# luo-yining/CFDBench

Hardware: NVIDIA H100
Metric: fno_rollout_steps_per_sec (higher is better)
Workload: dtype bf16

## Files before the change

cfdbench_b200/_lib.py:

```python
from __future__ import annotations

import ctypes as C
import os

_HERE = os.path.dirname(os.path.abspath(__file__))
LIB_PATH = os.path.join(_HERE, "libcfdbench_b200.so")

FNO_MAX_LAYERS = 8
ABI_VERSION = 4
ACT_F32, ACT_BF16 = 0, 1
EPI_GELU, EPI_GELU_SAVE_PRE, EPI_MUL_DGELU, EPI_PLAIN = 0, 1, 2, 3


class FnoWeights(C.Structure):
    _fields_ = [
        ("n_layers", C.c_int32),
        ("n_case_params", C.c_int32),
        ("fc0_w", C.c_void_p),
        ("fc0_b", C.c_void_p),
        ("spec_wk", C.c_void_p * FNO_MAX_LAYERS),
        ("w0t", C.c_void_p * FNO_MAX_LAYERS),
        ("w0_b", C.c_void_p * FNO_MAX_LAYERS),
        ("fc1_w", C.c_void_p),
        ("fc1_b", C.c_void_p),
# ... 64 lines not shown
    "fno_bwd_partials_bytes": (C.c_size_t, []),
    "fno_mode_mix_image": (C.c_int, [_P, _P, _P, _I, _P]),
    "fno_block_fused": (C.c_int, [_P, _P, _P, _P, _P, _I, _P]),
    "fno_pack_spectral_weights": (C.c_int, [_P, _P, _P, _I, _P]),
    "fno_unpack_spectral_grads": (C.c_int, [_P, _P, _P, _P]),
    "fno_mix_operand_bytes": (C.c_size_t, []),
    "fno_pack_mix_operand": (C.c_int, [_P, _P, _P]),
    "fno_pack_mix_operand_from_weights": (C.c_int, [_P, _P, _P, _I, _P]),
    "fno_lift_fwd": (C.c_int, [_P, _P, _P, C.POINTER(FnoWeights), _P, _I, _I, _P]),
    "fno_spectral_dft_fwd": (C.c_int, [_P, _P, _I, _I, _F, _F, _P]),
    "fno_mode_mix": (C.c_int, [_P, _P, _P, _I, _P]),
    "fno_spectral_inv_kx": (C.c_int, [_P, _P, _I, _F, _F, _P]),
    "fno_block_out": (C.c_int, [_I, _P, _P, _P, _P, _P, _P, _P, _I, _I, _P]),
    "fno_block_fwd": (C.c_int, [C.POINTER(FnoWeights), _I, _P, _P, _P, C.POINTER(FnoWorkspace), _I, _I, _P]),
    "fno_project_fwd": (C.c_int, [_P, _P, C.POINTER(FnoWeights), _P, _I, _I, _P]),
    "fno_forward": (C.c_int, [C.POINTER(FnoWeights), _P, _P, _P, _P, C.POINTER(FnoWorkspace), _I, _I, _P]),
    "fno_rollout": (C.c_int, [C.POINTER(FnoWeights), _P, _P, _P, _P, _I, C.POINTER(FnoWorkspace), _I, _I, _P]),
    "fno_rollout_host": (C.c_int, [C.POINTER(FnoWeights), _P, _P, _P, _P, _I, C.POINTER(FnoWorkspace), _P, _I, _I, _P]),
    "fno_rollout_host_scratch_bytes": (C.c_size_t, [_I, _I, _I]),
    "fno_multistep_metrics": (C.c_int, [_P, _P, _P, _P, _I, _I, _P]),
    "fno_gather_batch": (C.c_int, [_P, _P, _P, _P, _P, _I, _I, _I, _P, _P, _P, _P, _P]),
    "fno_loss_scratch_bytes": (C.c_size_t, []),
    "fno_loss_fwd": (C.c_int, [_P, _P, C.c_size_t, _P, _P, _P]),
    "fno_loss_bwd": (C.c_int, [_P, _P, _P, _P, _P, C.c_size_t, _P]),
    "fno_adam_step": (C.c_int, [C.POINTER(FnoAdamTensors), C.c_float, C.c_float, C.c_float, C.c_float, C.c_float,
                                C.c_int64, _P]),
    "fno_forward_train": (C.c_int, [C.POINTER(FnoWeights), _P, _P, _P, _P, C.POINTER(FnoTrainSaved),
                                    C.POINTER(FnoWorkspace), _I, _I, _P]),
    "fno_backward": (C.c_int, [C.POINTER(FnoWeights), C.POINTER(FnoWeightsBwd), _P, _P, _P, _P,
                               C.POINTER(FnoTrainSaved), C.POINTER(FnoGrads), C.POINTER(FnoBwdScratch),
# ... 55 lines not shown
```

cfdbench_b200/build.py:

```python
from __future__ import annotations

import hashlib
import os
import subprocess
import sys
import time

HERE = os.path.dirname(os.path.abspath(__file__))
CSRC = os.path.join(HERE, "csrc")
OUT = os.path.join(HERE, "libcfdbench_b200.so")
STAMP = os.path.join(HERE, ".build_stamp")
SOURCES = ["fno_abi.cu", "fno_dft_fwd.cu", "fno_dft_fwd_tc.cu", "fno_mode_mix.cu", "fno_block_tc.cu", "fno_block_fused.cu", "fno_pointwise.cu", "fno_project_tc.cu", "fno_project_bwd_tc.cu",
           "fno_backward.cu", "fno_metrics.cu", "fno_train_step.cu", "fno_grid.cu"]
NVCC_FLAGS = ["-std=c++17", "-O3", "-lineinfo", "-gencode", "arch=compute_90a,code=sm_90a",
              "-Xcompiler", "-fPIC"]


def _nvcc() -> str:
    for cand in (os.environ.get("NVCC"), "/usr/local/cuda/bin/nvcc"):
        if cand and os.path.exists(cand):
            return cand
    return "nvcc"


def _fingerprint() -> str:
    h = hashlib.sha256()
    for root in (CSRC, os.path.join(os.path.dirname(HERE), "include")):
# ... 52 lines not shown
```

cfdbench_b200/csrc/fno_abi.cu:

```cuda
#include <stdio.h>
#include <string.h>

#include "../../include/cfdbench_b200.h"
#include "fno_common.cuh"

namespace fno {
cudaError_t launch_dft_fwd(const void*, void*, int, float, float, cudaStream_t);
cudaError_t launch_mode_mix(const void*, const void*, void*, void*, int, cudaStream_t);
cudaError_t launch_block_fused(const void*, const void*, const float*, const float*, void*, int, cudaStream_t);
size_t ym_image_bytes(int);
cudaError_t launch_pack_spectral(const void*, const void*, void*, int, cudaStream_t);
cudaError_t launch_unpack_spectral(const void*, void*, void*, cudaStream_t);
cudaError_t launch_dft_fwd_tc(const void*, void*, int, float, float, cudaStream_t);
cudaError_t launch_pack_mix_operand(const void*, void*, cudaStream_t);
cudaError_t launch_pack_mix_operand_direct(const void*, const void*, void*, int, cudaStream_t);
size_t mix_operand_bytes();
cudaError_t launch_gather_batch(const void*, const void*, const float*, const int*, const long long*, int, int, int, float*,
                                float*, float*, float*, cudaStream_t);
cudaError_t launch_loss_fwd(const float*, const float*, size_t, float*, float*, cudaStream_t);
cudaError_t launch_loss_bwd(const float*, const float*, const float*, const float*, float*, size_t, cudaStream_t);
size_t loss_scratch_bytes();
cudaError_t launch_adam_step(const fno_adam_tensors*, float, float, float, float, float, long long, cudaStream_t);
cudaError_t launch_inv_kx(const void*, void*, int, float, float, cudaStream_t);
template <typename TAct>
cudaError_t launch_block_tc(int, const void*, const void*, const float*, const float*, void*, float*, const float*, int,
                            cudaStream_t);
template <typename TAct>
cudaError_t launch_lift(const float*, const float*, const float*, const float*, const float*, const float*,
                        const float*, void*, int, int, cudaStream_t);
template <typename TAct>
cudaError_t launch_project_tc(const void*, const float*, const float*, const float*, const float*, const float*,
                              float*, int, cudaStream_t);
int project_bwd_rows_max();
int project_bwd_row();
cudaError_t launch_reduce_partials(const float*, int, int, float*, int, float*, int, float*, int, int, cudaStream_t);
template <typename TAct>
cudaError_t launch_project_bwd_tc(const void*, const float*, const float*, const float*, const float*, const float*, const float*,
                                  float*, float*, float*, int*, int, cudaStream_t);
template <typename TP, typename TQ, int NJ, int NI>
cudaError_t launch_chan_outer(const void*, const void*, float*, int*, int, cudaStream_t);
cudaError_t launch_multistep_metrics(const float*, const float*, const float*, float*, int, int, cudaStream_t);
cudaError_t launch_spectral_wgrad(const void*, const void*, void*, int, cudaStream_t);
cudaError_t launch_lift_bwd(const float*, const float*, const float*, const float*, const float*, const float*,
                            float*, float*, float*, int, int, cudaStream_t);
cudaError_t launch_lift_bwd_data(const float*, const float*, float*, float*, int, int, cudaStream_t);
bool grid_ok(int, int);
void grid_tables_release(int);
// ... 178 lines not shown
  }
  FNO_TRY(fno_mode_mix(ws->xm, w->spec_wk[layer], ws->ym, batch, stream));
  const float inv = 1.f / static_cast<float>(kHW);
  FNO_TRY(fno_spectral_inv_kx(ws->ym, ws->z, batch, inv, 2.f * inv, stream));
  return fno_block_out(pre_out ? FNO_EPI_GELU_SAVE_PRE : FNO_EPI_GELU, ws->z, act_in, w->w0t[layer], w->w0_b[layer],
                       act_out, pre_out, nullptr, batch, act_dtype, stream);
}

int fno_project_fwd(const void* act_in, const float* mask, const fno_weights* w, float* preds, int batch,
                    int act_dtype, void* stream) {
  if (!act_in || !mask || !w || !preds || batch <= 0 || bad_dtype(act_dtype))
    return fail(kErrArg, "fno_project_fwd: bad argument");
  cudaError_t e =
      act_dtype == FNO_ACT_F32
          ? launch_project_tc<float>(act_in, w->fc1_w, w->fc1_b, w->fc2_w, w->fc2_b, mask, preds, batch, S(stream))
          : launch_project_tc<__nv_bfloat16>(act_in, w->fc1_w, w->fc1_b, w->fc2_w, w->fc2_b, mask, preds, batch, S(stream));
  FNO_CUDA(e, "project_kernel");
  return kOk;
}

int fno_forward(const fno_weights* w, const float* inputs, const float* mask, const float* case_params,
                float* preds, const fno_workspace* ws, int batch, int act_dtype, void* stream) {
  if (!w || !ws || !ws->act[0] || !ws->act[1] || !ws->xm) return fail(kErrArg, "fno_forward: bad workspace");
  if (!(act_dtype == FNO_ACT_BF16 && ws->ym_img) && (!ws->ym || !ws->z)) return fail(kErrArg, "fno_forward: bad workspace");
  if (w->n_layers < 1 || w->n_layers > FNO_MAX_LAYERS) return fail(kErrUnsupported, "fno_forward: n_layers out of range");
  FNO_TRY(fno_lift_fwd(inputs, mask, case_params, w, ws->act[0], batch, act_dtype, stream));
  int cur = 0;
  for (int l = 0; l < w->n_layers; ++l) {
    FNO_TRY(fno_block_fwd(w, l, ws->act[cur], ws->act[cur ^ 1], nullptr, ws, batch, act_dtype, stream));
    cur ^= 1;
  }
  return fno_project_fwd(ws->act[cur], mask, w, preds, batch, act_dtype, stream);
}

int fno_rollout(const fno_weights* w, const float* inputs, const float* mask, const float* case_params,
                float* preds_seq, int steps, const fno_workspace* ws, int batch, int act_dtype, void* stream) {
  if (steps < 0 || !preds_seq) return fail(kErrArg, "fno_rollout: bad argument");
  const size_t frame = static_cast<size_t>(batch) * 2 * kHW;
  const float* cur = inputs;
  for (int s = 0; s < steps; ++s) {
    float* nxt = preds_seq + static_cast<size_t>(s) * frame;
    FNO_TRY(fno_forward(w, cur, mask, case_params, nxt, ws, batch, act_dtype, stream));
    cur = nxt;
  }
  return kOk;
}

size_t fno_rollout_host_scratch_bytes(int batch, int n_case_params, int steps) {
  const size_t b = static_cast<size_t>(batch);
  return (b * 2 * kHW + b * kHW + static_cast<size_t>(steps) * b * 2 * kHW) * sizeof(float) +
         ((b * n_case_params * sizeof(float) + 255) / 256) * 256;
}

int fno_rollout_host(const fno_weights* w, const float* inputs_host, const float* mask_host,
                     const float* case_params_host, float* preds_seq_host, int steps, const fno_workspace* ws,
                     void* dev_io, int batch, int act_dtype, void* stream) {
  if (!w || !inputs_host || !mask_host || !preds_seq_host || !dev_io || batch <= 0 || steps <= 0)
    return fail(kErrArg, "fno_rollout_host: bad argument");
// ... 399 lines not shown
```

cfdbench_b200/csrc/fno_block_fused.cu:

```cuda
#include "fno_common.cuh"
#include "tc_common.cuh"
#include "tc_tma.cuh"
#include <math.h>
#include <string.h>

namespace fno {

constexpr int kFzRows = 16;
constexpr int kFzChunks = kH / kFzRows;
constexpr int kFzWgRows = kFzRows / 2;
constexpr int kFzThreads = 9 * 32;
constexpr int kFzProdWarp = 8;
constexpr int kZK = 2 * kM2;
constexpr int kImgK = 2 * kKX;
constexpr size_t kYmImgBytes = 147456;
constexpr uint32_t kFzStage = 4 * 6144;
constexpr int kFzFFloats = 2 * (2 * kFzRows) * kImgK;
constexpr int kFzEFloats = 2 * kW * kZK;
constexpr uint32_t kFzZtFloats = kC * kZK;
constexpr uint32_t kLboF = (2 * kFzRows / 8) * 128;
constexpr uint32_t kLboE = (kW / 8) * 128;
constexpr uint32_t kLboO = (kC / 8) * 128;
constexpr uint32_t kFzBoxW = kW, kFzBoxH = 1, kFzBoxC = kC;
constexpr uint32_t kFzRowBytes = kFzBoxW * kFzBoxH * kFzBoxC * 2;
// ... 7 lines not shown
  alignas(1024) unsigned char x[2][kFzXSlots][kFzRowBytes];
  alignas(1024) unsigned char st[2][2][kFzRowBytes];
  alignas(128) unsigned char y[2][kFzStage];
  alignas(128) float zt[kFzRows][2][kFzZtFloats];
  alignas(128) float f_hi[kFzFFloats / 2];
  alignas(128) float f_lo[kFzFFloats / 2];
  alignas(128) float e_hi[kFzEFloats / 2];
  alignas(128) float e_lo[kFzEFloats / 2];
  alignas(128) unsigned char w0[3][kFzW0Bytes];
  alignas(16) float bias[kC];
  alignas(8) uint64_t y_full[2], y_free[2];
  alignas(8) uint64_t x_full[2][kFzXSlots];
};
static_assert(sizeof(FzSmem) <= 232448, "block_fused_kernel: shared memory over the per-block opt-in limit");

__device__ __forceinline__ uint32_t sw128_bf16_offset(int line, int e) {
  return static_cast<uint32_t>(line * 128 + ((((e >> 3) ^ line) & 7) << 4) + (e & 7) * 2);
}

__global__ void __launch_bounds__(kFzThreads, 1)
    block_fused_kernel(const __grid_constant__ CUtensorMap x_map, const __grid_constant__ CUtensorMap out_map,
                       const unsigned char* __restrict__ img, const float* __restrict__ w0t,
                       const float* __restrict__ bias, const float* __restrict__ etab, const float* __restrict__ ftab,
                       int batch) {
  extern __shared__ __align__(1024) unsigned char smem_raw[];
  FzSmem& sm = *reinterpret_cast<FzSmem*>(smem_raw);
  if ((smem_u32(smem_raw) & 1023u) != 0) __trap();
  const int tid = threadIdx.x, lane = tid & 31, warp = tc::warp_index_uniform();
  const int chunk = blockIdx.x % kFzChunks, b0 = blockIdx.x / kFzChunks, bstride = gridDim.x / kFzChunks;
  const int n_units = b0 < batch ? (batch - b0 + bstride - 1) / bstride : 0;

  if (tid == 0) {
    for (int i = 0; i < 2; ++i) {
      mbar_init(&sm.y_full[i], 1);
// ... 260 lines not shown
```

cfdbench_b200/csrc/fno_project_tc.cu:

```cuda
#include "fno_common.cuh"
#include "tc_common.cuh"

namespace fno {

constexpr int kPtWG = 4;
constexpr int kPtThreads = 128 * kPtWG;
constexpr int kPtM = kW;
constexpr uint32_t kPtLboA = (kPtM / 8) * 128;
constexpr uint32_t kPtLboB = (kProj / 8) * 128;
constexpr int kPtTilesPerSample = kH;
constexpr int kPtReps = kPtM * (kC / 4) / 128;

struct PtSmem {
  alignas(128) float w_hi[kProj * kC];
  alignas(128) float w_lo[kProj * kC];
  alignas(128) float a_hi[kPtWG][kPtM * kC];
  alignas(128) float a_lo[kPtWG][kPtM * kC];
  alignas(16) float4 w2q[kProj / 2];
  alignas(16) float2 b1p[kProj / 2];
};

template <typename TAct>
struct PtRegs {
  TAct v[kPtReps][4];
};

template <typename TAct>
__device__ __forceinline__ void pt_prefetch(PtRegs<TAct>& r, const TAct* __restrict__ a, int tile, int t) {
  const int b = tile / kPtTilesPerSample, p0 = (tile % kPtTilesPerSample) * kPtM;
#pragma unroll
  for (int rep = 0; rep < kPtReps; ++rep) {
    const int task = rep * 128 + t;
    const int m = task & (kPtM - 1), kq = task >> 6;
    const TAct* src = a + (static_cast<size_t>(b) * kC + 4 * kq) * kHW + p0 + m;
#pragma unroll
    for (int c = 0; c < 4; ++c) r.v[rep][c] = __ldg(src + static_cast<size_t>(c) * kHW);
  }
}

__device__ __forceinline__ float pt_to_float(float v) { return v; }
__device__ __forceinline__ float pt_to_float(__nv_bfloat16 v) { return __bfloat162float(v); }

template <typename TAct>
__device__ __forceinline__ void pt_split_store(const PtRegs<TAct>& r, float* a_hi, float* a_lo, int t) {
#pragma unroll
  for (int rep = 0; rep < kPtReps; ++rep) {
    const int task = rep * 128 + t;
    const int m = task & (kPtM - 1), kq = task >> 6;
    float hi[4], lo[4];
#pragma unroll
    for (int c = 0; c < 4; ++c) {
      const float x = pt_to_float(r.v[rep][c]);
      if constexpr (sizeof(TAct) == 4) tc::split_tf32(x, hi[c], lo[c]);
      else hi[c] = x;
    }
    const uint32_t off = tc::kmajor_offset(m, 4 * kq, kPtM) / 4;
    *reinterpret_cast<float4*>(a_hi + off) = make_float4(hi[0], hi[1], hi[2], hi[3]);
    if constexpr (sizeof(TAct) == 4) *reinterpret_cast<float4*>(a_lo + off) = make_float4(lo[0], lo[1], lo[2], lo[3]);
  }
}

template <typename TAct>
__global__ void __launch_bounds__(kPtThreads, 1)
    project_tc_kernel(const TAct* __restrict__ a, const float* __restrict__ w1, const float* __restrict__ b1,
                      const float* __restrict__ w2, const float* __restrict__ b2, const float* __restrict__ mask,
                      float* __restrict__ preds, int n_tiles) {
  constexpr bool kBf16 = sizeof(TAct) == 2;
  extern __shared__ __align__(1024) unsigned char smem_raw[];
  PtSmem& sm = *reinterpret_cast<PtSmem*>(smem_raw);
  const int tid = threadIdx.x, lane = tid & 31;
  const int wg = tc::warp_index_uniform() >> 2, t = tid & 127, wq = (tid >> 5) & 3;

  for (int e = tid; e < kProj * kC; e += kPtThreads) {
    const int j = e / kC, i = e % kC;
    float hi, lo;
    tc::split_tf32(w1[e], hi, lo);
    const uint32_t off = tc::kmajor_offset(j, i, kProj) / 4;
    sm.w_hi[off] = hi;
    sm.w_lo[off] = lo;
  }
  if (tid < kProj / 2) {
    sm.w2q[tid] = make_float4(w2[2 * tid], w2[kProj + 2 * tid], w2[2 * tid + 1], w2[kProj + 2 * tid + 1]);
// ... 10 lines not shown
  float* a_lo = sm.a_lo[wg];
  PtRegs<TAct> regs;
  if (first < n_tiles) pt_prefetch<TAct>(regs, a, first, t);
  for (int tile = first; tile < n_tiles; tile += stride) {
    pt_split_store<TAct>(regs, a_hi, a_lo, t);
    tc::fence_proxy_async_smem();
    tc::named_barrier(1 + wg, 128);
    if (tile + stride < n_tiles) pt_prefetch<TAct>(regs, a, tile + stride, t);
    float acc[64];
    tc::wg_fence();
    {
      const uint32_t a_s[3] = {tc::smem_addr(a_hi), tc::smem_addr(a_lo), tc::smem_addr(a_hi)};
      const uint32_t b_s[3] = {tc::smem_addr(sm.w_hi), tc::smem_addr(sm.w_hi), tc::smem_addr(sm.w_lo)};
#pragma unroll
      for (int pass = 0; pass < 3; ++pass) {
        if (kBf16 && pass == 1) continue;
#pragma unroll
        for (int ks = 0; ks < kC / 8; ++ks)
          tc::wg_tf32_ss_n128(acc, tc::make_smem_desc(a_s[pass] + ks * 2 * kPtLboA, kPtLboA, 128),
                              tc::make_smem_desc(b_s[pass] + ks * 2 * kPtLboB, kPtLboB, 128), (pass | ks) ? 1u : 0u);
      }
    }
    tc::wg_commit();
    tc::wg_wait<0>();
    tc::wg_fence_acc(acc);
    const int b = tile / kPtTilesPerSample, p0 = (tile % kPtTilesPerSample) * kPtM;
#pragma unroll
    for (int hh = 0; hh < 2; ++hh) {
      float2 out = make_float2(0.f, 0.f);
#pragma unroll
      for (int i0 = 0; i0 < 16; i0 += 8) {
        float2 g[8];
#pragma unroll
        for (int i = 0; i < 8; ++i) {
          const float2 bb = sm.b1p[4 * (i0 + i) + (lane & 3)];
          g[i] = make_float2(acc[4 * (i0 + i) + 2 * hh] + bb.x, acc[4 * (i0 + i) + 2 * hh + 1] + bb.y);
        }
        if constexpr (kBf16) {
          gelu_erf2_deg5_batch<8>(g);
        } else {
#pragma unroll
          for (int i = 0; i < 8; ++i) g[i] = gelu_erf2(g[i]);
        }
#pragma unroll
        for (int i = 0; i < 8; ++i) {
          const float4 wq4 = sm.w2q[4 * (i0 + i) + (lane & 3)];
          out = ffma2(make_float2(g[i].x, g[i].x), make_float2(wq4.x, wq4.y), out);
          out = ffma2(make_float2(g[i].y, g[i].y), make_float2(wq4.z, wq4.w), out);
        }
      }
      out.x += __shfl_xor_sync(0xffffffffu, out.x, 1);
      out.y += __shfl_xor_sync(0xffffffffu, out.y, 1);
      out.x += __shfl_xor_sync(0xffffffffu, out.x, 2);
      out.y += __shfl_xor_sync(0xffffffffu, out.y, 2);
      if ((lane & 3) == 0) {
        const int pix = p0 + 16 * wq + (lane >> 2) + 8 * hh;
        const float mk = __ldg(mask + static_cast<size_t>(b) * kHW + pix);
        preds[(static_cast<size_t>(b) * 2 + 0) * kHW + pix] = (b2x + out.x) * mk;
// ... 8 lines not shown
                              const float* mask, float* preds, int batch, cudaStream_t stream) {
  auto kern = project_tc_kernel<TAct>;
  constexpr size_t smem = sizeof(PtSmem);
  static PerDeviceLaunch pd;
  int n_sm = 0;
  cudaError_t e0 = per_device_setup(kern, smem, pd, &n_sm);
  if (e0 != cudaSuccess) return e0;
  const int n_tiles = batch * kPtTilesPerSample;
  const int want = (n_tiles + kPtWG - 1) / kPtWG;
  const int grid = want < n_sm ? want : n_sm;
  return launch_chained(kern, dim3(grid), dim3(kPtThreads), smem, stream, static_cast<const TAct*>(a), w1, b1, w2, b2,
                        mask, preds, n_tiles);
}
template cudaError_t launch_project_tc<float>(const void*, const float*, const float*, const float*, const float*,
                                              const float*, float*, int, cudaStream_t);
template cudaError_t launch_project_tc<__nv_bfloat16>(const void*, const float*, const float*, const float*,
                                                      const float*, const float*, float*, int, cudaStream_t);

}
```

cfdbench_b200/csrc/tc_common.cuh:

```cuda
#pragma once
#include <cuda_runtime.h>
#include <stdint.h>

namespace fno {
namespace tc {

__device__ __forceinline__ uint32_t smem_addr(const void* p) {
  return static_cast<uint32_t>(__cvta_generic_to_shared(p));
}

__device__ __forceinline__ int warp_index_uniform() {
  return __shfl_sync(0xffffffffu, static_cast<int>(threadIdx.x >> 5), 0);
}

__device__ __forceinline__ void named_barrier(int id, int count) {
  asm volatile("bar.sync %0, %1;" ::"r"(id), "r"(count) : "memory");
}

__device__ __forceinline__ void fence_proxy_async_smem() {
  asm volatile("fence.proxy.async.shared::cta;" ::: "memory");
}

__device__ __forceinline__ uint64_t make_smem_desc(uint32_t saddr, uint32_t lbo_bytes, uint32_t sbo_bytes) {
  uint64_t d = 0;
// ... 47 lines not shown
  asm volatile(
      "{\n.reg .pred p;\nsetp.ne.b32 p, %38, 0;\n"
      "wgmma.mma_async.sync.aligned.m64n72k16.f32.bf16.bf16 {%0, %1, %2, %3, %4, %5, %6, %7, %8, %9, %10, %11, %12, %13, %14, %15, %16, %17, %18, %19, %20, %21, %22, %23, %24, %25, %26, %27, %28, %29, %30, %31, %32, %33, %34, %35}, %36, %37, p, 1, 1, 0, 0;\n}\n"
      : "+f"(d[0]), "+f"(d[1]), "+f"(d[2]), "+f"(d[3]), "+f"(d[4]), "+f"(d[5]), "+f"(d[6]), "+f"(d[7]), "+f"(d[8]), "+f"(d[9]), "+f"(d[10]), "+f"(d[11]), "+f"(d[12]), "+f"(d[13]), "+f"(d[14]), "+f"(d[15]), "+f"(d[16]), "+f"(d[17]), "+f"(d[18]), "+f"(d[19]), "+f"(d[20]), "+f"(d[21]), "+f"(d[22]), "+f"(d[23]), "+f"(d[24]), "+f"(d[25]), "+f"(d[26]), "+f"(d[27]), "+f"(d[28]), "+f"(d[29]), "+f"(d[30]), "+f"(d[31]), "+f"(d[32]), "+f"(d[33]), "+f"(d[34]), "+f"(d[35])
      : "l"(a), "l"(b), "r"(acc)
      : "memory");
}
__device__ __forceinline__ void wg_bf16_ss_n32_mn_a(float* d, uint64_t a, uint64_t b, uint32_t acc) {
  asm volatile(
      "{\n.reg .pred p;\nsetp.ne.b32 p, %18, 0;\n"
      "wgmma.mma_async.sync.aligned.m64n32k16.f32.bf16.bf16 {%0, %1, %2, %3, %4, %5, %6, %7, %8, %9, %10, %11, %12, %13, %14, %15}, %16, %17, p, 1, 1, 1, 0;\n}\n"
      : "+f"(d[0]), "+f"(d[1]), "+f"(d[2]), "+f"(d[3]), "+f"(d[4]), "+f"(d[5]), "+f"(d[6]), "+f"(d[7]), "+f"(d[8]), "+f"(d[9]), "+f"(d[10]), "+f"(d[11]), "+f"(d[12]), "+f"(d[13]), "+f"(d[14]), "+f"(d[15])
      : "l"(a), "l"(b), "r"(acc)
      : "memory");
}
__device__ __forceinline__ void wg_tf32_rs_n32(float* d, const uint32_t* a, uint64_t b, uint32_t acc) {
  asm volatile(
      "{\n.reg .pred p;\nsetp.ne.b32 p, %21, 0;\n"
      "wgmma.mma_async.sync.aligned.m64n32k8.f32.tf32.tf32 {%0, %1, %2, %3, %4, %5, %6, %7, %8, %9, %10, %11, %12, %13, %14, %15}, {%16, %17, %18, %19}, %20, p, 1, 1;\n}\n"
      : "+f"(d[0]), "+f"(d[1]), "+f"(d[2]), "+f"(d[3]), "+f"(d[4]), "+f"(d[5]), "+f"(d[6]), "+f"(d[7]), "+f"(d[8]), "+f"(d[9]), "+f"(d[10]), "+f"(d[11]), "+f"(d[12]), "+f"(d[13]), "+f"(d[14]), "+f"(d[15])
      : "r"(a[0]), "r"(a[1]), "r"(a[2]), "r"(a[3]), "l"(b), "r"(acc)
      : "memory");
}
__device__ __forceinline__ void wg_tf32_rs_n64(float* d, const uint32_t* a, uint64_t b, uint32_t acc) {
  asm volatile(
      "{\n.reg .pred p;\nsetp.ne.b32 p, %37, 0;\n"
      "wgmma.mma_async.sync.aligned.m64n64k8.f32.tf32.tf32 {%0, %1, %2, %3, %4, %5, %6, %7, %8, %9, %10, %11, %12, %13, %14, %15, %16, %17, %18, %19, %20, %21, %22, %23, %24, %25, %26, %27, %28, %29, %30, %31}, {%32, %33, %34, %35}, %36, p, 1, 1;\n}\n"
      : "+f"(d[0]), "+f"(d[1]), "+f"(d[2]), "+f"(d[3]), "+f"(d[4]), "+f"(d[5]), "+f"(d[6]), "+f"(d[7]), "+f"(d[8]), "+f"(d[9]), "+f"(d[10]), "+f"(d[11]), "+f"(d[12]), "+f"(d[13]), "+f"(d[14]), "+f"(d[15]), "+f"(d[16]), "+f"(d[17]), "+f"(d[18]), "+f"(d[19]), "+f"(d[20]), "+f"(d[21]), "+f"(d[22]), "+f"(d[23]), "+f"(d[24]), "+f"(d[25]), "+f"(d[26]), "+f"(d[27]), "+f"(d[28]), "+f"(d[29]), "+f"(d[30]), "+f"(d[31])
      : "r"(a[0]), "r"(a[1]), "r"(a[2]), "r"(a[3]), "l"(b), "r"(acc)
      : "memory");
// ... 16 lines not shown
```

cfdbench_b200/csrc/tc_tma.cuh:

```cuda
#pragma once
#include "fno_common.cuh"
#include <cuda.h>

namespace fno {

__device__ __forceinline__ void tma_load_2d(void* dst, const CUtensorMap* tm, int c0, int c1, uint64_t* bar) {
  asm volatile("cp.async.bulk.tensor.2d.shared::cluster.global.mbarrier::complete_tx::bytes [%0], [%1, {%2, %3}], [%4];" ::"r"(
                   smem_u32(dst)),
               "l"(tm), "r"(c0), "r"(c1), "r"(smem_u32(bar))
               : "memory");
}
__device__ __forceinline__ void tma_load_3d(void* dst, const CUtensorMap* tm, int c0, int c1, int c2, uint64_t* bar) {
  asm volatile(
      "cp.async.bulk.tensor.3d.shared::cluster.global.mbarrier::complete_tx::bytes [%0], [%1, {%2, %3, %4}], [%5];" ::"r"(
          smem_u32(dst)),
      "l"(tm), "r"(c0), "r"(c1), "r"(c2), "r"(smem_u32(bar))
      : "memory");
}
__device__ __forceinline__ void tma_store_3d(const CUtensorMap* tm, const void* src, int c0, int c1, int c2) {
  asm volatile("cp.async.bulk.tensor.3d.global.shared::cta.bulk_group [%0, {%2, %3, %4}], [%1];" ::"l"(tm),
               "r"(smem_u32(src)), "r"(c0), "r"(c1), "r"(c2)
               : "memory");
}
__device__ __forceinline__ void bulk_commit_group() { asm volatile("cp.async.bulk.commit_group;" ::: "memory"); }
template <int kPending>
__device__ __forceinline__ void bulk_wait_group_read() {
  asm volatile("cp.async.bulk.wait_group.read %0;" ::"n"(kPending) : "memory");
}
template <int kPending>
__device__ __forceinline__ void bulk_wait_group() {
  asm volatile("cp.async.bulk.wait_group %0;" ::"n"(kPending) : "memory");
}

typedef CUresult (*TmaEncodeFn)(CUtensorMap*, CUtensorMapDataType, cuuint32_t, void*, const cuuint64_t*, const cuuint64_t*,
                                const cuuint32_t*, const cuuint32_t*, CUtensorMapInterleave, CUtensorMapSwizzle,
                                CUtensorMapL2promotion, CUtensorMapFloatOOBfill);
inline cudaError_t tma_encode_fn(TmaEncodeFn* out) {
// ... 41 lines not shown
```

include/cfdbench_b200.h:

```cpp
#ifndef CFDBENCH_B200_H_
#define CFDBENCH_B200_H_

#include <stddef.h>
#include <stdint.h>

#ifdef __cplusplus
extern "C" {
#endif

#define FNO_ABI_VERSION 4
#define FNO_MAX_LAYERS 8

enum { FNO_ACT_F32 = 0, FNO_ACT_BF16 = 1 };
enum { FNO_EPI_GELU = 0, FNO_EPI_GELU_SAVE_PRE = 1, FNO_EPI_MUL_DGELU = 2, FNO_EPI_PLAIN = 3 };

typedef struct fno_weights {
  int32_t n_layers;
  int32_t n_case_params;
  const float* fc0_w;
  const float* fc0_b;
  const void* spec_wk[FNO_MAX_LAYERS];
  const float* w0t[FNO_MAX_LAYERS];
  const float* w0_b[FNO_MAX_LAYERS];
  const float* fc1_w;
// ... 32 lines not shown
                 void* act_out, int batch, int act_dtype, void* stream);

int fno_spectral_dft_fwd(const void* act_in, void* xm, int batch, int act_dtype, float s0, float s1, void* stream);
int fno_mode_mix(const void* xm, const void* wop, void* ym, int batch, void* stream);
int fno_spectral_inv_kx(const void* ym, void* z, int batch, float s0, float s1, void* stream);
int fno_block_out(int epilogue, const void* z, const void* act_in, const float* w0t, const float* bias, void* act_out,
                  float* pre_out, const float* pre_in, int batch, int act_dtype, void* stream);
int fno_mode_mix_image(const void* xm, const void* wop, void* ym_img, int batch, void* stream);
int fno_block_fused(const void* ym_img, const void* act_in_bf16, const float* w0t, const float* bias, void* act_out_bf16,
                    int batch, void* stream);
int fno_block_fwd(const fno_weights* w, int layer, const void* act_in, void* act_out, float* pre_out,
                  const fno_workspace* ws, int batch, int act_dtype, void* stream);

int fno_project_fwd(const void* act_in, const float* mask, const fno_weights* w, float* preds, int batch,
                    int act_dtype, void* stream);

int fno_forward(const fno_weights* w, const float* inputs, const float* mask, const float* case_params,
                float* preds, const fno_workspace* ws, int batch, int act_dtype, void* stream);

int fno_rollout(const fno_weights* w, const float* inputs, const float* mask, const float* case_params,
                float* preds_seq, int steps, const fno_workspace* ws, int batch, int act_dtype, void* stream);

int fno_rollout_host(const fno_weights* w, const float* inputs_host, const float* mask_host,
                     const float* case_params_host, float* preds_seq_host, int steps, const fno_workspace* ws,
                     void* dev_io, int batch, int act_dtype, void* stream);
size_t fno_rollout_host_scratch_bytes(int batch, int n_case_params, int steps);


typedef struct fno_train_saved {
  void* act[FNO_MAX_LAYERS + 1];
// ... 103 lines not shown
```

Before: 1211.

## Fuse bf16 projection with next-step lift in rollout via new wgmma kernel

Adds a bf16 projection kernel that uses TMA-loaded activation rows and bf16 wgmma with a 3-term split of fc1 weights. In rollout, the kernel also computes the next step's lifted activation directly from its predictions, removing a separate lift launch and the round trip through global memory for each step. The bf16 path of the old TF32 projection kernel is removed and replaced by the new kernel. This adds kernel complexity, and the triple-bf16 weight split risks small numeric differences.

```diff
diff --git a/cfdbench_b200/_lib.py b/cfdbench_b200/_lib.py
--- a/cfdbench_b200/_lib.py
+++ b/cfdbench_b200/_lib.py
@@ -102,6 +102,7 @@
     "fno_block_out": (C.c_int, [_I, _P, _P, _P, _P, _P, _P, _P, _I, _I, _P]),
     "fno_block_fwd": (C.c_int, [C.POINTER(FnoWeights), _I, _P, _P, _P, C.POINTER(FnoWorkspace), _I, _I, _P]),
     "fno_project_fwd": (C.c_int, [_P, _P, C.POINTER(FnoWeights), _P, _I, _I, _P]),
+    "fno_project_lift_fwd": (C.c_int, [_P, _P, _P, C.POINTER(FnoWeights), _P, _P, _I, _P]),
     "fno_forward": (C.c_int, [C.POINTER(FnoWeights), _P, _P, _P, _P, C.POINTER(FnoWorkspace), _I, _I, _P]),
     "fno_rollout": (C.c_int, [C.POINTER(FnoWeights), _P, _P, _P, _P, _I, C.POINTER(FnoWorkspace), _I, _I, _P]),
     "fno_rollout_host": (C.c_int, [C.POINTER(FnoWeights), _P, _P, _P, _P, _I, C.POINTER(FnoWorkspace), _P, _I, _I, _P]),
diff --git a/cfdbench_b200/build.py b/cfdbench_b200/build.py
--- a/cfdbench_b200/build.py
+++ b/cfdbench_b200/build.py
@@ -10,7 +10,7 @@
 CSRC = os.path.join(HERE, "csrc")
 OUT = os.path.join(HERE, "libcfdbench_b200.so")
 STAMP = os.path.join(HERE, ".build_stamp")
-SOURCES = ["fno_abi.cu", "fno_dft_fwd.cu", "fno_dft_fwd_tc.cu", "fno_mode_mix.cu", "fno_block_tc.cu", "fno_block_fused.cu", "fno_pointwise.cu", "fno_project_tc.cu", "fno_project_bwd_tc.cu",
+SOURCES = ["fno_abi.cu", "fno_dft_fwd.cu", "fno_dft_fwd_tc.cu", "fno_mode_mix.cu", "fno_block_tc.cu", "fno_block_fused.cu", "fno_pointwise.cu", "fno_project_tc.cu", "fno_project_bf16.cu", "fno_project_bwd_tc.cu",
            "fno_backward.cu", "fno_metrics.cu", "fno_train_step.cu", "fno_grid.cu"]
 NVCC_FLAGS = ["-std=c++17", "-O3", "-lineinfo", "-gencode", "arch=compute_90a,code=sm_90a",
               "-Xcompiler", "-fPIC"]
diff --git a/cfdbench_b200/csrc/fno_abi.cu b/cfdbench_b200/csrc/fno_abi.cu
--- a/cfdbench_b200/csrc/fno_abi.cu
+++ b/cfdbench_b200/csrc/fno_abi.cu
@@ -31,6 +31,9 @@
 template <typename TAct>
 cudaError_t launch_project_tc(const void*, const float*, const float*, const float*, const float*, const float*,
                               float*, int, cudaStream_t);
+cudaError_t launch_project_bf16(const void*, const float*, const float*, const float*, const float*, const float*, float*,
+                                void*, const float*, const float*, const float*, const float*, const float*, int, int,
+                                cudaStream_t);
 int project_bwd_rows_max();
 int project_bwd_row();
 cudaError_t launch_reduce_partials(const float*, int, int, float*, int, float*, int, float*, int, int, cudaStream_t);
@@ -239,22 +242,57 @@
   cudaError_t e =
       act_dtype == FNO_ACT_F32
           ? launch_project_tc<float>(act_in, w->fc1_w, w->fc1_b, w->fc2_w, w->fc2_b, mask, preds, batch, S(stream))
-          : launch_project_tc<__nv_bfloat16>(act_in, w->fc1_w, w->fc1_b, w->fc2_w, w->fc2_b, mask, preds, batch, S(stream));
-  FNO_CUDA(e, "project_kernel");
-  return kOk;
-}
-
-int fno_forward(const fno_weights* w, const float* inputs, const float* mask, const float* case_params,
-                float* preds, const fno_workspace* ws, int batch, int act_dtype, void* stream) {
-  if (!w || !ws || !ws->act[0] || !ws->act[1] || !ws->xm) return fail(kErrArg, "fno_forward: bad workspace");
-  if (!(act_dtype == FNO_ACT_BF16 && ws->ym_img) && (!ws->ym || !ws->z)) return fail(kErrArg, "fno_forward: bad workspace");
-  if (w->n_layers < 1 || w->n_layers > FNO_MAX_LAYERS) return fail(kErrUnsupported, "fno_forward: n_layers out of range");
-  FNO_TRY(fno_lift_fwd(inputs, mask, case_params, w, ws->act[0], batch, act_dtype, stream));
-  int cur = 0;
+          : launch_project_bf16(act_in, w->fc1_w, w->fc1_b, w->fc2_w, w->fc2_b, mask, preds, nullptr, nullptr, nullptr,
+                                nullptr, nullptr, nullptr, 0, batch, S(stream));
+  FNO_CUDA(e, act_dtype == FNO_ACT_F32 ? "project_tc_kernel" : "project_bf16_kernel");
+  return kOk;
+}
+
+int fno_project_lift_fwd(const void* act_in, const float* mask, const float* case_params, const fno_weights* w, float* preds,
+                         void* act_next, int batch, void* stream) {
+  if (!act_in || !mask || !w || !preds || !act_next || batch <= 0 || !w->gx || !w->gy)
+    return fail(kErrArg, "fno_project_lift_fwd: bad argument");
+  if (w->n_case_params < 0 || w->n_case_params > kMaxCaseParams)
+    return fail(kErrArg, "fno_project_lift_fwd: n_case_params out of range");
+  if (w->n_case_params > 0 && !case_params) return fail(kErrArg, "fno_project_lift_fwd: case_params is null");
+  if ((reinterpret_cast<uintptr_t>(act_in) | reinterpret_cast<uintptr_t>(act_next)) & 15)
+    return fail(kErrArg, "fno_project_lift_fwd: act_in / act_next must be 16-byte aligned");
+  const size_t bytes = fno_act_bytes(batch, FNO_ACT_BF16);
+  const char *in = static_cast<const char*>(act_in), *nx = static_cast<const char*>(act_next);
+  if (in < nx + bytes && nx < in + bytes) return fail(kErrArg, "fno_project_lift_fwd: act_in and act_next overlap");
+  FNO_CUDA(launch_project_bf16(act_in, w->fc1_w, w->fc1_b, w->fc2_w, w->fc2_b, mask, preds, act_next, case_params, w->fc0_w,
+                               w->fc0_b, w->gx, w->gy, w->n_case_params, batch, S(stream)),
+           "project_bf16_kernel(lift)");
+  return kOk;
+}
+
+static int check_forward_workspace(const char* what, const fno_weights* w, const fno_workspace* ws, int act_dtype) {
+  char msg[128];
+  snprintf(msg, sizeof(msg), "%s: bad workspace", what);
+  if (!w || !ws || !ws->act[0] || !ws->act[1] || !ws->xm) return fail(kErrArg, msg);
+  if (!(act_dtype == FNO_ACT_BF16 && ws->ym_img) && (!ws->ym || !ws->z)) return fail(kErrArg, msg);
+  snprintf(msg, sizeof(msg), "%s: n_layers out of range", what);
+  if (w->n_layers < 1 || w->n_layers > FNO_MAX_LAYERS) return fail(kErrUnsupported, msg);
+  return kOk;
+}
+
+static int forward_layers(const fno_weights* w, const fno_workspace* ws, int a0, int batch, int act_dtype, void* stream,
+                          int* out) {
+  int cur = a0;
   for (int l = 0; l < w->n_layers; ++l) {
     FNO_TRY(fno_block_fwd(w, l, ws->act[cur], ws->act[cur ^ 1], nullptr, ws, batch, act_dtype, stream));
     cur ^= 1;
   }
+  *out = cur;
+  return kOk;
+}
+
+int fno_forward(const fno_weights* w, const float* inputs, const float* mask, const float* case_params,
+                float* preds, const fno_workspace* ws, int batch, int act_dtype, void* stream) {
+  FNO_TRY(check_forward_workspace("fno_forward", w, ws, act_dtype));
+  FNO_TRY(fno_lift_fwd(inputs, mask, case_params, w, ws->act[0], batch, act_dtype, stream));
+  int cur = 0;
+  FNO_TRY(forward_layers(w, ws, 0, batch, act_dtype, stream, &cur));
   return fno_project_fwd(ws->act[cur], mask, w, preds, batch, act_dtype, stream);
 }
 
@@ -262,11 +300,26 @@
                 float* preds_seq, int steps, const fno_workspace* ws, int batch, int act_dtype, void* stream) {
   if (steps < 0 || !preds_seq) return fail(kErrArg, "fno_rollout: bad argument");
   const size_t frame = static_cast<size_t>(batch) * 2 * kHW;
-  const float* cur = inputs;
+  if (act_dtype != FNO_ACT_BF16) {
+    const float* cur = inputs;
+    for (int s = 0; s < steps; ++s) {
+      float* nxt = preds_seq + static_cast<size_t>(s) * frame;
+      FNO_TRY(fno_forward(w, cur, mask, case_params, nxt, ws, batch, act_dtype, stream));
+      cur = nxt;
+    }
+    return kOk;
+  }
+  if (steps == 0) return kOk;
+  FNO_TRY(check_forward_workspace("fno_rollout", w, ws, act_dtype));
+  FNO_TRY(fno_lift_fwd(inputs, mask, case_params, w, ws->act[0], batch, act_dtype, stream));
+  int a0 = 0;
   for (int s = 0; s < steps; ++s) {
     float* nxt = preds_seq + static_cast<size_t>(s) * frame;
-    FNO_TRY(fno_forward(w, cur, mask, case_params, nxt, ws, batch, act_dtype, stream));
-    cur = nxt;
+    int cur = 0;
+    FNO_TRY(forward_layers(w, ws, a0, batch, act_dtype, stream, &cur));
+    if (s + 1 == steps) return fno_project_fwd(ws->act[cur], mask, w, nxt, batch, act_dtype, stream);
+    FNO_TRY(fno_project_lift_fwd(ws->act[cur], mask, case_params, w, nxt, ws->act[cur ^ 1], batch, stream));
+    a0 = cur ^ 1;
   }
   return kOk;
 }
diff --git a/cfdbench_b200/csrc/fno_block_fused.cu b/cfdbench_b200/csrc/fno_block_fused.cu
--- a/cfdbench_b200/csrc/fno_block_fused.cu
+++ b/cfdbench_b200/csrc/fno_block_fused.cu
@@ -45,10 +45,6 @@
 };
 static_assert(sizeof(FzSmem) <= 232448, "block_fused_kernel: shared memory over the per-block opt-in limit");
 
-__device__ __forceinline__ uint32_t sw128_bf16_offset(int line, int e) {
-  return static_cast<uint32_t>(line * 128 + ((((e >> 3) ^ line) & 7) << 4) + (e & 7) * 2);
-}
-
 __global__ void __launch_bounds__(kFzThreads, 1)
     block_fused_kernel(const __grid_constant__ CUtensorMap x_map, const __grid_constant__ CUtensorMap out_map,
                        const unsigned char* __restrict__ img, const float* __restrict__ w0t,
diff --git a/cfdbench_b200/csrc/fno_project_bf16.cu b/cfdbench_b200/csrc/fno_project_bf16.cu
--- /dev/null
+++ b/cfdbench_b200/csrc/fno_project_bf16.cu
@@ -0,0 +1,264 @@
+#include "fno_common.cuh"
+#include "tc_common.cuh"
+#include "tc_tma.cuh"
+#include <type_traits>
+
+namespace fno {
+
+constexpr int kPjWG = 4;
+constexpr int kPjThreads = 128 * kPjWG;
+constexpr int kPjTilesPerSample = kH;
+constexpr uint32_t kPjBoxW = kW, kPjBoxH = 1, kPjBoxC = kC;
+constexpr uint32_t kPjRowBytes = kPjBoxW * kPjBoxH * kPjBoxC * 2;
+constexpr int kPjXSlots = 4;
+constexpr uint32_t kPjW1Bytes = kProj * kC * 2;
+constexpr uint32_t kPjLboW = (kProj / 8) * 128;
+
+__host__ __device__ constexpr int pj_x_slot(int n) { return n % kPjXSlots; }
+__host__ __device__ constexpr uint32_t pj_x_parity(int n) { return static_cast<uint32_t>(n / kPjXSlots) & 1u; }
+
+struct PjSmem {
+  alignas(1024) unsigned char x[kPjWG][kPjXSlots][kPjRowBytes];
+  alignas(1024) unsigned char st[kPjWG][2][kPjRowBytes];
+  alignas(128) unsigned char w1[3][kPjW1Bytes];
+  alignas(16) float4 w2q[kProj / 2];
+  alignas(16) float2 b1p[kProj / 2];
+  alignas(16) float4 lw4[kC];
+  float lwx[kC];
+  float lwp[kC][kMaxCaseParams];
+  float lb[kC];
+  float gx[kH], gy[kW];
+  float base[kPjWG][2][kC];
+  alignas(8) uint64_t x_full[kPjWG][kPjXSlots];
+};
+static_assert(sizeof(PjSmem) <= 232448, "project_bf16_kernel: shared memory over the per-block opt-in limit");
+
+template <bool kLift>
+__global__ void __launch_bounds__(kPjThreads, 1)
+    project_bf16_kernel(const __grid_constant__ CUtensorMap x_map, const __grid_constant__ CUtensorMap out_map,
+                        const float* __restrict__ w1, const float* __restrict__ b1, const float* __restrict__ w2,
+                        const float* __restrict__ b2, const float* __restrict__ mask, float* __restrict__ preds,
+                        const float* __restrict__ params, const float* __restrict__ fc0_w, const float* __restrict__ fc0_b,
+                        const float* __restrict__ gx, const float* __restrict__ gy, int p, int n_tiles) {
+  extern __shared__ __align__(1024) unsigned char smem_raw[];
+  PjSmem& sm = *reinterpret_cast<PjSmem*>(smem_raw);
+  if ((smem_u32(smem_raw) & 1023u) != 0) __trap();
+  const int tid = threadIdx.x, lane = tid & 31;
+  const int wg = tc::warp_index_uniform() >> 2, t = tid & 127, wq = (tid >> 5) & 3, q = lane & 3;
+
+  if (tid == 0) {
+    for (int g = 0; g < kPjWG; ++g)
+      for (int s = 0; s < kPjXSlots; ++s) mbar_init(&sm.x_full[g][s], 1);
+    fence_mbar_init();
+  }
+  for (int e = tid; e < kProj * kC; e += kPjThreads) {
+    const int j = e / kC, i = e % kC;
+    const float v = w1[e];
+    const __nv_bfloat16 t1 = __float2bfloat16_rn(v);
+    const float r1 = v - __bfloat162float(t1);
+    const __nv_bfloat16 t2 = __float2bfloat16_rn(r1);
+    const __nv_bfloat16 t3 = __float2bfloat16_rn(r1 - __bfloat162float(t2));
+    const uint32_t off = static_cast<uint32_t>(((i >> 3) * (kProj / 8) + (j >> 3)) * 128 + (j & 7) * 16 + (i & 7) * 2);
+    *reinterpret_cast<__nv_bfloat16*>(sm.w1[0] + off) = t1;
+    *reinterpret_cast<__nv_bfloat16*>(sm.w1[1] + off) = t2;
+    *reinterpret_cast<__nv_bfloat16*>(sm.w1[2] + off) = t3;
+  }
+  if (tid < kProj / 2) {
+    sm.w2q[tid] = make_float4(w2[2 * tid], w2[kProj + 2 * tid], w2[2 * tid + 1], w2[kProj + 2 * tid + 1]);
+    sm.b1p[tid] = make_float2(b1[2 * tid], b1[2 * tid + 1]);
+  }
+  if constexpr (kLift) {
+    const int nin = 5 + p;
+    if (tid < kC) {
+      sm.lw4[tid] = make_float4(fc0_w[tid * nin + 0], fc0_w[tid * nin + 1], fc0_w[tid * nin + 2], fc0_w[tid * nin + 4]);
+      sm.lwx[tid] = fc0_w[tid * nin + 3];
+      for (int k = 0; k < p; ++k) sm.lwp[tid][k] = fc0_w[tid * nin + 5 + k];
+      sm.lb[tid] = fc0_b[tid];
+    }
+    if (tid < kH) sm.gx[tid] = gx[tid];
+    if (tid < kW) sm.gy[tid] = gy[tid];
+  }
+  const float b2x = b2[0], b2y = b2[1];
+  tc::fence_proxy_async_smem();
+  __syncthreads();
+  pdl_wait();
+  pdl_launch_dependents();
+
+  const int first = blockIdx.x * kPjWG + wg, stride = gridDim.x * kPjWG;
+  const int n_fills = first < n_tiles ? (n_tiles - first + stride - 1) / stride : 0;
+  auto x_fill = [&](int n) {
+    const int tile = first + n * stride, s = pj_x_slot(n);
+    mbar_expect_tx(&sm.x_full[wg][s], kPjRowBytes);
+    tma_load_3d(sm.x[wg][s], &x_map, 0, tile % kPjTilesPerSample, (tile / kPjTilesPerSample) * kC, &sm.x_full[wg][s]);
+  };
+  if (t == 0)
+    for (int n = 0; n < kPjXSlots && n < n_fills; ++n) x_fill(n);
+  const uint32_t w1_s = tc::smem_addr(sm.w1[0]);
+  const int m0 = 16 * wq + (lane >> 2);
+  auto issue_half = [&](float (&acc)[32], int n, int hf) {
+    const uint32_t a_x = tc::smem_addr(sm.x[wg][pj_x_slot(n)]);
+    tc::wg_fence();
+#pragma unroll
+    for (int term = 0; term < 3; ++term)
+#pragma unroll
+      for (int ks = 0; ks < kC / 16; ++ks)
+        tc::wg_bf16_ss_n64_mn_a(acc, tc::make_smem_desc_sw128_mn(a_x + ks * 2048),
+                                tc::make_smem_desc(w1_s + hf * (kProj / 2 / 8) * 128 + term * kPjW1Bytes + ks * 2 * kPjLboW,
+                                                   kPjLboW, 128),
+                                (term | ks) ? 1u : 0u);
+    tc::wg_commit();
+  };
+  auto epilogue_half = [&](const float (&acc)[32], int hf, float2 (&out)[2]) {
+#pragma unroll
+    for (int hh = 0; hh < 2; ++hh) {
+      float2 g[8];
+#pragma unroll
+      for (int i = 0; i < 8; ++i) {
+        const float2 bb = sm.b1p[4 * (8 * hf + i) + q];
+        g[i] = make_float2(acc[4 * i + 2 * hh] + bb.x, acc[4 * i + 2 * hh + 1] + bb.y);
+      }
+      gelu_erf2_deg5_batch<8>(g);
+#pragma unroll
+      for (int i = 0; i < 8; ++i) {
+        const float4 wq4 = sm.w2q[4 * (8 * hf + i) + q];
+        out[hh] = ffma2(make_float2(g[i].x, g[i].x), make_float2(wq4.x, wq4.y), out[hh]);
+        out[hh] = ffma2(make_float2(g[i].y, g[i].y), make_float2(wq4.z, wq4.w), out[hh]);
+      }
+    }
+  };
+  auto lift_params = [&](int n) {
+    const int b = (first + n * stride) / kPjTilesPerSample;
+    return lane < p ? __ldg(params + static_cast<size_t>(b) * p + lane) : 0.f;
+  };
+  auto lift_base = [&](int n, float pv) {
+    const int h = (first + n * stride) % kPjTilesPerSample;
+    float cb = sm.lb[lane];
+    for (int k = 0; k < p; ++k) cb = fmaf(sm.lwp[lane][k], __shfl_sync(0xffffffffu, pv, k), cb);
+    sm.base[wg][n & 1][lane] = fmaf(sm.lwx[lane], sm.gx[h], cb);
+  };
+  if (n_fills == 0) return;
+  if constexpr (kLift) {
+    if (wq == 0) lift_base(0, lift_params(0));
+    tc::named_barrier(1 + wg, 128);
+  }
+  uint32_t soff[2][2];
+#pragma unroll
+  for (int hh = 0; hh < 2; ++hh)
+#pragma unroll
+    for (int kk = 0; kk < 2; ++kk) soff[hh][kk] = sw128_bf16_offset(q + 4 * kk, m0 + 8 * hh);
+
+  float acc0[32], acc1[32];
+  mbar_wait(&sm.x_full[wg][pj_x_slot(0)], pj_x_parity(0));
+  issue_half(acc0, 0, 0);
+  issue_half(acc1, 0, 1);
+  auto tile_step = [&](int n, auto next) {
+    constexpr bool kNext = decltype(next)::value;
+    const int tile = first + n * stride, b = tile / kPjTilesPerSample, h = tile % kPjTilesPerSample;
+    float mk[2];
+#pragma unroll
+    for (int hh = 0; hh < 2; ++hh) mk[hh] = __ldg(mask + static_cast<size_t>(b) * kHW + h * kW + m0 + 8 * hh);
+    float pv_next = 0.f;
+    if (kLift && kNext && wq == 0) pv_next = lift_params(n + 1);
+    float2 out[2] = {make_float2(0.f, 0.f), make_float2(0.f, 0.f)};
+    tc::wg_wait<1>();
+    tc::wg_fence_acc(acc0);
+    epilogue_half(acc0, 0, out);
+    if constexpr (kNext) {
+      mbar_wait(&sm.x_full[wg][pj_x_slot(n + 1)], pj_x_parity(n + 1));
+      issue_half(acc0, n + 1, 0);
+      tc::wg_wait<1>();
+    } else {
+      tc::wg_wait<0>();
+    }
+    tc::wg_fence_acc(acc1);
+    epilogue_half(acc1, 1, out);
+    float u[2], v[2];
+#pragma unroll
+    for (int hh = 0; hh < 2; ++hh) {
+      out[hh].x += __shfl_xor_sync(0xffffffffu, out[hh].x, 1);
+      out[hh].y += __shfl_xor_sync(0xffffffffu, out[hh].y, 1);
+      out[hh].x += __shfl_xor_sync(0xffffffffu, out[hh].x, 2);
+      out[hh].y += __shfl_xor_sync(0xffffffffu, out[hh].y, 2);
+      const int pix = h * kW + m0 + 8 * hh;
+      u[hh] = (b2x + out[hh].x) * mk[hh];
+      v[hh] = (b2y + out[hh].y) * mk[hh];
+      if (q == 0) {
+        preds[(static_cast<size_t>(b) * 2 + 0) * kHW + pix] = u[hh];
+        preds[(static_cast<size_t>(b) * 2 + 1) * kHW + pix] = v[hh];
+      }
+    }
+    if constexpr (kLift) {
+      unsigned char* stile = sm.st[wg][n & 1];
+      const float* base = sm.base[wg][n & 1];
+      const float yw[2] = {sm.gy[m0], sm.gy[m0 + 8]};
+#pragma unroll
+      for (int k = 0; k < kC / 4; ++k) {
+        const int c = q + 4 * k;
+        const float4 wt = sm.lw4[c];
+        const float bc = base[c];
+#pragma unroll
+        for (int hh = 0; hh < 2; ++hh) {
+          const float r = fmaf(wt.x, u[hh], fmaf(wt.y, v[hh], fmaf(wt.z, mk[hh], fmaf(wt.w, yw[hh], bc))));
+          *reinterpret_cast<__nv_bfloat16*>(stile + soff[hh][k & 1] + 1024 * (k >> 1)) = __float2bfloat16_rn(r);
+        }
+      }
+      if (kNext && wq == 0) lift_base(n + 1, pv_next);
+      tc::fence_proxy_async_smem();
+      if (t == 0) bulk_wait_group_read<0>();
+    }
+    tc::named_barrier(1 + wg, 128);
+    if (t == 0) {
+      if constexpr (kLift) {
+        tma_store_3d(&out_map, sm.st[wg][n & 1], 0, h, b * kC);
+        bulk_commit_group();
+      }
+      if (n + kPjXSlots < n_fills) x_fill(n + kPjXSlots);
+    }
+    if constexpr (kNext) issue_half(acc1, n + 1, 1);
+  };
+  for (int n = 0; n + 1 < n_fills; ++n) tile_step(n, std::true_type());
+  tile_step(n_fills - 1, std::false_type());
+  if constexpr (kLift) {
+    if (t == 0) bulk_wait_group<0>();
+  }
+}
+
+template <bool kLift>
+static cudaError_t launch_project_bf16_kernel(const CUtensorMap& x_map, const CUtensorMap& out_map, const float* w1,
+                                              const float* b1, const float* w2, const float* b2, const float* mask,
+                                              float* preds, const float* params, const float* fc0_w, const float* fc0_b,
+                                              const float* gx, const float* gy, int p, int batch, cudaStream_t stream) {
+  auto kern = project_bf16_kernel<kLift>;
+  constexpr size_t smem = sizeof(PjSmem);
+  static PerDeviceLaunch pd;
+  int n_sm = 0;
+  cudaError_t e = per_device_setup(kern, smem, pd, &n_sm);
+  if (e != cudaSuccess) return e;
+  const int n_tiles = batch * kPjTilesPerSample;
+  const int want = (n_tiles + kPjWG - 1) / kPjWG;
+  const int grid = want < n_sm ? want : n_sm;
+  return launch_chained(kern, dim3(grid), dim3(kPjThreads), smem, stream, x_map, out_map, w1, b1, w2, b2, mask, preds,
+                        params, fc0_w, fc0_b, gx, gy, p, n_tiles);
+}
+
+cudaError_t launch_project_bf16(const void* a, const float* w1, const float* b1, const float* w2, const float* b2,
+                                const float* mask, float* preds, void* a_next, const float* params, const float* fc0_w,
+                                const float* fc0_b, const float* gx, const float* gy, int p, int batch,
+                                cudaStream_t stream) {
+  if (p < 0 || p > kMaxCaseParams) return cudaErrorInvalidValue;
+  if ((reinterpret_cast<uintptr_t>(a) & 15) || (reinterpret_cast<uintptr_t>(a_next) & 15))
+    return cudaErrorMisalignedAddress;
+  CUtensorMap x_map, out_map;
+  const uint64_t planes = static_cast<uint64_t>(batch) * kC;
+  cudaError_t e = make_tma_map_3d(&x_map, CU_TENSOR_MAP_DATA_TYPE_BFLOAT16, 2, a, kW, kH, planes, kPjBoxW, kPjBoxH, kPjBoxC);
+  if (e != cudaSuccess) return e;
+  if (!a_next)
+    return launch_project_bf16_kernel<false>(x_map, x_map, w1, b1, w2, b2, mask, preds, nullptr, nullptr, nullptr, nullptr,
+                                             nullptr, 0, batch, stream);
+  e = make_tma_map_3d(&out_map, CU_TENSOR_MAP_DATA_TYPE_BFLOAT16, 2, a_next, kW, kH, planes, kPjBoxW, kPjBoxH, kPjBoxC);
+  if (e != cudaSuccess) return e;
+  return launch_project_bf16_kernel<true>(x_map, out_map, w1, b1, w2, b2, mask, preds, params, fc0_w, fc0_b, gx, gy, p,
+                                          batch, stream);
+}
+
+}
diff --git a/cfdbench_b200/csrc/fno_project_tc.cu b/cfdbench_b200/csrc/fno_project_tc.cu
--- a/cfdbench_b200/csrc/fno_project_tc.cu
+++ b/cfdbench_b200/csrc/fno_project_tc.cu
@@ -38,9 +38,6 @@
   }
 }
 
-__device__ __forceinline__ float pt_to_float(float v) { return v; }
-__device__ __forceinline__ float pt_to_float(__nv_bfloat16 v) { return __bfloat162float(v); }
-
 template <typename TAct>
 __device__ __forceinline__ void pt_split_store(const PtRegs<TAct>& r, float* a_hi, float* a_lo, int t) {
 #pragma unroll
@@ -50,13 +47,11 @@
     float hi[4], lo[4];
 #pragma unroll
     for (int c = 0; c < 4; ++c) {
-      const float x = pt_to_float(r.v[rep][c]);
-      if constexpr (sizeof(TAct) == 4) tc::split_tf32(x, hi[c], lo[c]);
-      else hi[c] = x;
+      tc::split_tf32(r.v[rep][c], hi[c], lo[c]);
     }
     const uint32_t off = tc::kmajor_offset(m, 4 * kq, kPtM) / 4;
     *reinterpret_cast<float4*>(a_hi + off) = make_float4(hi[0], hi[1], hi[2], hi[3]);
-    if constexpr (sizeof(TAct) == 4) *reinterpret_cast<float4*>(a_lo + off) = make_float4(lo[0], lo[1], lo[2], lo[3]);
+    *reinterpret_cast<float4*>(a_lo + off) = make_float4(lo[0], lo[1], lo[2], lo[3]);
   }
 }
 
@@ -65,7 +60,6 @@
     project_tc_kernel(const TAct* __restrict__ a, const float* __restrict__ w1, const float* __restrict__ b1,
                       const float* __restrict__ w2, const float* __restrict__ b2, const float* __restrict__ mask,
                       float* __restrict__ preds, int n_tiles) {
-  constexpr bool kBf16 = sizeof(TAct) == 2;
   extern __shared__ __align__(1024) unsigned char smem_raw[];
   PtSmem& sm = *reinterpret_cast<PtSmem*>(smem_raw);
   const int tid = threadIdx.x, lane = tid & 31;
@@ -106,7 +100,6 @@
       const uint32_t b_s[3] = {tc::smem_addr(sm.w_hi), tc::smem_addr(sm.w_hi), tc::smem_addr(sm.w_lo)};
 #pragma unroll
       for (int pass = 0; pass < 3; ++pass) {
-        if (kBf16 && pass == 1) continue;
 #pragma unroll
         for (int ks = 0; ks < kC / 8; ++ks)
           tc::wg_tf32_ss_n128(acc, tc::make_smem_desc(a_s[pass] + ks * 2 * kPtLboA, kPtLboA, 128),
@@ -128,12 +121,8 @@
           const float2 bb = sm.b1p[4 * (i0 + i) + (lane & 3)];
           g[i] = make_float2(acc[4 * (i0 + i) + 2 * hh] + bb.x, acc[4 * (i0 + i) + 2 * hh + 1] + bb.y);
         }
-        if constexpr (kBf16) {
-          gelu_erf2_deg5_batch<8>(g);
-        } else {
 #pragma unroll
-          for (int i = 0; i < 8; ++i) g[i] = gelu_erf2(g[i]);
-        }
+        for (int i = 0; i < 8; ++i) g[i] = gelu_erf2(g[i]);
 #pragma unroll
         for (int i = 0; i < 8; ++i) {
           const float4 wq4 = sm.w2q[4 * (i0 + i) + (lane & 3)];
@@ -172,7 +161,5 @@
 }
 template cudaError_t launch_project_tc<float>(const void*, const float*, const float*, const float*, const float*,
                                               const float*, float*, int, cudaStream_t);
-template cudaError_t launch_project_tc<__nv_bfloat16>(const void*, const float*, const float*, const float*,
-                                                      const float*, const float*, float*, int, cudaStream_t);
 
 }
diff --git a/cfdbench_b200/csrc/tc_common.cuh b/cfdbench_b200/csrc/tc_common.cuh
--- a/cfdbench_b200/csrc/tc_common.cuh
+++ b/cfdbench_b200/csrc/tc_common.cuh
@@ -85,6 +85,14 @@
       : "l"(a), "l"(b), "r"(acc)
       : "memory");
 }
+__device__ __forceinline__ void wg_bf16_ss_n64_mn_a(float* d, uint64_t a, uint64_t b, uint32_t acc) {
+  asm volatile(
+      "{\n.reg .pred p;\nsetp.ne.b32 p, %34, 0;\n"
+      "wgmma.mma_async.sync.aligned.m64n64k16.f32.bf16.bf16 {%0, %1, %2, %3, %4, %5, %6, %7, %8, %9, %10, %11, %12, %13, %14, %15, %16, %17, %18, %19, %20, %21, %22, %23, %24, %25, %26, %27, %28, %29, %30, %31}, %32, %33, p, 1, 1, 1, 0;\n}\n"
+      : "+f"(d[0]), "+f"(d[1]), "+f"(d[2]), "+f"(d[3]), "+f"(d[4]), "+f"(d[5]), "+f"(d[6]), "+f"(d[7]), "+f"(d[8]), "+f"(d[9]), "+f"(d[10]), "+f"(d[11]), "+f"(d[12]), "+f"(d[13]), "+f"(d[14]), "+f"(d[15]), "+f"(d[16]), "+f"(d[17]), "+f"(d[18]), "+f"(d[19]), "+f"(d[20]), "+f"(d[21]), "+f"(d[22]), "+f"(d[23]), "+f"(d[24]), "+f"(d[25]), "+f"(d[26]), "+f"(d[27]), "+f"(d[28]), "+f"(d[29]), "+f"(d[30]), "+f"(d[31])
+      : "l"(a), "l"(b), "r"(acc)
+      : "memory");
+}
 __device__ __forceinline__ void wg_tf32_rs_n32(float* d, const uint32_t* a, uint64_t b, uint32_t acc) {
   asm volatile(
       "{\n.reg .pred p;\nsetp.ne.b32 p, %21, 0;\n"
diff --git a/cfdbench_b200/csrc/tc_tma.cuh b/cfdbench_b200/csrc/tc_tma.cuh
--- a/cfdbench_b200/csrc/tc_tma.cuh
+++ b/cfdbench_b200/csrc/tc_tma.cuh
@@ -21,6 +21,9 @@
   asm volatile("cp.async.bulk.tensor.3d.global.shared::cta.bulk_group [%0, {%2, %3, %4}], [%1];" ::"l"(tm),
                "r"(smem_u32(src)), "r"(c0), "r"(c1), "r"(c2)
                : "memory");
+}
+__device__ __forceinline__ uint32_t sw128_bf16_offset(int line, int e) {
+  return static_cast<uint32_t>(line * 128 + ((((e >> 3) ^ line) & 7) << 4) + (e & 7) * 2);
 }
 __device__ __forceinline__ void bulk_commit_group() { asm volatile("cp.async.bulk.commit_group;" ::: "memory"); }
 template <int kPending>
diff --git a/include/cfdbench_b200.h b/include/cfdbench_b200.h
--- a/include/cfdbench_b200.h
+++ b/include/cfdbench_b200.h
@@ -70,6 +70,8 @@
 
 int fno_project_fwd(const void* act_in, const float* mask, const fno_weights* w, float* preds, int batch,
                     int act_dtype, void* stream);
+int fno_project_lift_fwd(const void* act_in, const float* mask, const float* case_params, const fno_weights* w, float* preds,
+                         void* act_next, int batch, void* stream);
 
 int fno_forward(const fno_weights* w, const float* inputs, const float* mask, const float* case_params,
                 float* preds, const fno_workspace* ws, int batch, int act_dtype, void* stream);
```

Measured after the change: 1211 (median of 6 runs). Within noise of the previous version (+0.0%).
